# lingo-db/lingo-db

Measured on AMD Instinct MI355X. Metric: tpch_sf100_geomean_ms, lower is better.
Workload: dtype int64/int128 decimal

## Files before the change

lingo-db_amd/csrc/ldb_core.hip:

```cpp
#include "ldb_internal.h"
#include "ldb_device.h"
#include "ldb_chain.h"
#include <algorithm>
#include <cstdlib>
#include <memory>

static thread_local char g_err[1024] = "";
void ldb_set_error(const char* fmt, ...) {
   va_list ap;
   va_start(ap, fmt);
   vsnprintf(g_err, sizeof(g_err), fmt, ap);
   va_end(ap);
}
extern "C" const char* ldb_gpu_last_error(void) { return g_err; }

#include <atomic>
#include <functional>
#include <mutex>
static std::mutex g_opt_mu;
static std::atomic<int64_t> g_option_epoch{0};
static std::unordered_map<std::string, int64_t> g_opts;
int64_t ldb_option(const char* name, int64_t dflt) {
   std::lock_guard<std::mutex> lock(g_opt_mu);
   auto it = g_opts.find(name);
   if (it != g_opts.end()) return it->second;
   std::string env = "LDB_";
   for (const char* c = name; *c; c++) env += (char) toupper((unsigned char) *c);
   int64_t v = dflt;
   if (const char* e = getenv(env.c_str())) v = atoll(e);
   g_opts[name] = v;
   return v;
}
extern "C" int32_t ldb_gpu_set_option(const char* name, int64_t value) {
   if (!name) LDB_FAIL(LDB_ERR_INVALID, "set_option: NULL name");
   static const char* known[] = {"jit", "jit_min_rows", "lazy_filter", "lazy_min_rows", "join_ordered", "join_chained", "gb_ordered", "gb_sorted", "zone_maps", "zone_min_rows", "gb_direct", "gb_wgs_per_cu", "gb_partition", "gb_partition_min_rows", "join_radix", "join_radix_min_rows", "join_radix_min_table_bytes", "join_radix_part_bytes", "probe_batch", "debug_check", "join_direct", "join_rank", "join_coarse", "dict_encode", "dict_min_rows", "comm_transport", "comm_timeout_ms", "desc_cache", "desc_cache_mb", "plan_replay", "scan_single_pass", "lazy_strings", "lazy_strings_min_rows", "gb_partition_wc", "join_radix_wc", "join_radix_lds", "gb_dense_out", "gb_partition_values", "join_pair32", "gb_dense_keys", "jit_async", "jit_threads", "jit_disk_cache", "join_all_match", "topk_short_select", "gb_fits64", "join_coarse_fine", "join_coarse_filtered", "compact_wide_tiles", "compact_max_words", "join_fuse_max_conjuncts", "join_coarse_finest", "jit_min_rows_like", "scan_split", "jit_share_compiles", "scan_strset_min_in"};
   bool ok = false;
   for (const char* k : known) ok |= strcmp(k, name) == 0;
   if (!ok) LDB_FAIL(LDB_ERR_INVALID, "set_option: unknown option '%s'", name);
   std::lock_guard<std::mutex> lock(g_opt_mu);
   g_opts[name] = value;
   g_option_epoch.fetch_add(1);
   return LDB_OK;
}
extern "C" int64_t ldb_gpu_get_option(const char* name) {
   if (!name) return -1;
   std::lock_guard<std::mutex> lock(g_opt_mu);
   auto it = g_opts.find(name);
   if (it != g_opts.end()) return it->second;
   std::string env = "LDB_";
   for (const char* c = name; *c; c++) env += (char) toupper((unsigned char) *c);
   if (const char* e = getenv(env.c_str())) return atoll(e);
   return -1;
}

double ldb_host_trace_threshold() {
   static const double thr = [] {
      const char* e = getenv("LDB_HOST_TRACE");
      return e && *e ? atof(e) : -1.0;
   }();
   return thr;
}
static size_t ldb_size_class(size_t bytes) {
   if (bytes <= 256) return 256;
   const int lg = 63 - __builtin_clzll((unsigned long long) (bytes - 1));
   const size_t step = (size_t) 1 << (lg >= 3 ? lg - 3 : 0);
   return (bytes + step - 1) / step * step;
}
static void ldb_cache_release(ldb_ctx* ctx) {
   for (auto& kv : ctx->parked)
      for (void* p : kv.second) (void) hipFreeAsync(p, ctx->stream);
   ctx->parked.clear();
   ctx->cache_bytes = 0;
}
int32_t ldb_dev_alloc(ldb_ctx* ctx, void** out, size_t bytes) {
   const size_t cls = ctx->cache_on ? ldb_size_class(bytes + 16) : bytes + 16;
   if (ctx->cache_on) {
      auto it = ctx->parked.find(cls);
      if (it != ctx->parked.end() && !it->second.empty()) {
         std::pop_heap(it->second.begin(), it->second.end(), std::greater<void*>());
         *out = it->second.back();
         it->second.pop_back();
         ctx->cache_bytes -= cls;
         ctx->live[*out] = cls;
         return LDB_OK;
      }
   }
   hipError_t e;
   {
      LdbSlow slow_("hipMallocAsync", cls);
      e = hipMallocAsync(out, cls, ctx->stream);
   }
   if (e != hipSuccess && ctx->cache_bytes) {
      (void) hipGetLastError();
      ldb_cache_release(ctx);
      (void) hipStreamSynchronize(ctx->stream);
      e = hipMallocAsync(out, cls, ctx->stream);
   }
   LDB_HIP(e);
   if (ctx->cache_on) ctx->live[*out] = cls;
   return LDB_OK;
}
void ldb_dev_free(ldb_ctx* ctx, void* p) {
   if (!p) return;
   auto dref = ctx->desc_blocks.find(p);
   if (dref != ctx->desc_blocks.end()) {
      if (dref->second > 0) dref->second--;
      else {
         ctx->desc_underflows++;
         if (ldb_host_trace_threshold() >= 0) fprintf(stderr, "[ldb] descriptor %p given back twice\n", p);
      }
      return;
   }
   if (!ctx->shared.empty()) {
      auto sh = ctx->shared.find(p);
      if (sh != ctx->shared.end()) {
         if (--sh->second == 0) ctx->shared.erase(sh);
         return;
      }
// ... 2038 lines not shown
```

lingo-db_amd/csrc/ldb_join.hip:

```cpp
#include "ldb_internal.h"
#include "ldb_join_kernel.h"
#include "ldb_jit.h"
#include <cmath>
#include "ldb_chain.h"
#include <algorithm>
#include <memory>

struct ldb_hashtable {
   ldb_ctx* ctx = nullptr;
   ldb_rel* build = nullptr;
   std::vector<ldb_colref> keys;
   uint64_t* slots = nullptr;
   uint64_t cap = 0;
   int32_t key32 = 0;
   int32_t unique = 0;
   int32_t ordered_slots = 0;
   int64_t kmin = 0, kmax = -1;
   uint64_t kmult = 0;
   uint32_t kmult32 = 0, ksh = 0;
   int32_t slot32 = 0;
   uint32_t* key_bits = nullptr;
   int32_t chained = 0;
   uint32_t* next = nullptr;
   int32_t direct = 0;
// ... 46 lines not shown
   __shared__ uint32_t s_prefix;
   if (threadIdx.x == 0) s_tile = atomicAdd(ticket, 1ull) - ticket_base;
   __syncthreads();
   const uint64_t tile = s_tile;
   const uint64_t base = tile * CHAIN_TILE + (uint64_t) threadIdx.x * CHAIN_ITEMS;
   uint32_t bits[CHAIN_ITEMS];
   uint32_t sum = 0;
#pragma unroll
   for (int k = 0; k < CHAIN_ITEMS; k++) {
      bits[k] = base + k < n_words ? (uint32_t) tab[base + k] : 0u;
      sum += (uint32_t) __popc(bits[k]);
   }
   uint32_t agg;
   uint32_t excl = d_block_scan256<uint32_t>(sum, s_wave, &agg);
   if (threadIdx.x < 64) {
      const uint32_t prefix = d_chain_prefix<uint32_t, 32>(status, tile, epoch, agg, threadIdx.x);
      if (threadIdx.x == 0) s_prefix = prefix;
   }
   __syncthreads();
   excl += s_prefix;
   if (total && tile == n_tiles - 1 && threadIdx.x == 0) *total = (unsigned long long) s_prefix + agg;
#pragma unroll
   for (int k = 0; k < CHAIN_ITEMS; k++) {
      if (base + k < n_words) tab[base + k] = (uint64_t) bits[k] | ((uint64_t) excl << 32);
      excl += (uint32_t) __popc(bits[k]);
   }
}
__global__ void k_join_probe_pairs(const DJoin* __restrict__ d);
__global__ void k_join_probe_pairs_count(const DJoin* __restrict__ d);
__global__ void k_join_probe_count(const DJoin* __restrict__ d);
__global__ void k_join_probe_exists(const DJoin* __restrict__ d);
__global__ void k_join_probe_unique(const DJoin* __restrict__ d);
__global__ void k_join_probe_markbuild(const DJoin* __restrict__ d);
__global__ void k_join_flags_bitmap(const uint8_t* __restrict__ flags, uint64_t n, int anti, uint64_t* __restrict__ bitmap, unsigned long long* __restrict__ counter) {
   join_flags_bitmap_body(flags, n, anti, bitmap, counter);
}
__global__ void k_join_flags_bitmap2(const uint8_t* __restrict__ flags, const uint8_t* __restrict__ not_flags, uint64_t n, uint64_t* __restrict__ bitmap, unsigned long long* __restrict__ counter) {
   join_flags_bitmap_body(flags, n, 0, bitmap, counter, not_flags);
}

static const char* JOIN_SPEC_SRC =
   "extern \"C\" __global__ void k_join_build_spec(const DJoin* __restrict__ d) { join_build_body(LDB_META, d); }\n"
   "extern \"C\" __global__ void k_join_probe_pairs_spec(const DJoin* __restrict__ d) { join_probe_pairs_body(LDB_META, d); }\n"
   "extern \"C\" __global__ void k_join_probe_pairs_count_spec(const DJoin* __restrict__ d) { join_probe_pairs_count_body(LDB_META, d); }\n"
   "extern \"C\" __global__ void k_join_probe_count_spec(const DJoin* __restrict__ d) { join_probe_count_body(LDB_META, d); }\n"
   "extern \"C\" __global__ void k_join_probe_exists_spec(const DJoin* __restrict__ d) { join_probe_exists_body(LDB_META, d); }\n"
   "extern \"C\" __global__ void k_join_probe_unique_spec(const DJoin* __restrict__ d) { join_probe_unique_body(LDB_META, d); }\n"
   "extern \"C\" __global__ void k_join_probe_markbuild_spec(const DJoin* __restrict__ d) { join_probe_markbuild_body(LDB_META, d); }\n";

typedef void (*join_kernel_t)(const DJoin*);
static int32_t launch_join(ldb_ctx* ctx, const DJoin* h, const DJoin* d, int grid, const char* prof_name, const char* spec_name, join_kernel_t generic) {
   hipFunction_t spec = nullptr;
   if (ldb_jit_wanted((int64_t) h->n_rows)) {
      auto meta = std::make_unique<DJoin>();
      memcpy(meta.get(), h, sizeof(DJoin));
      meta->n_rows = meta->cap = meta->slots = meta->out_probe = meta->out_build = meta->out_cap = 0;
      meta->counter = meta->bitmap = meta->mark = meta->mark2 = meta->match = meta->flags = 0;
      meta->kmin = meta->kmax = 0;
      meta->kmult = 0;
      meta->kmult32 = meta->ksh = 0;
      meta->key_bits = 0;
      meta->next = 0;
      meta->coarse = 0;
      meta->coarse_words = 0;
      ldb_jit_strip_keys(meta->bkeys);
      ldb_jit_strip_keys(meta->pkeys);
      for (int p = 0; p < LDB_MAX_PREDS; p++) ldb_jit_strip_pred(meta->ppreds[p]);
      for (int p = 0; p < LDB_MAX_M2PREDS; p++) ldb_jit_strip_pred(meta->m2preds[p]);
      for (int k = 0; k < LDB_MAX_RESID; k++) {
         ldb_jit_strip_col(meta->resid[k].pcol);
         ldb_jit_strip_col(meta->resid[k].bcol);
      }
      std::string why;
      std::string one;
      for (const char* line = JOIN_SPEC_SRC; *line;) {
         const char* nl = strchr(line, '\n');
         const size_t len = nl ? (size_t) (nl - line) + 1 : strlen(line);
         std::string l(line, len);
         if (l.find(std::string(" ") + spec_name + "(") != std::string::npos) one = l;
         line += len;
      }
      spec = ldb_jit_kernel(ctx->device, "ldb_join_kernel.h", "DJoin", one.empty() ? JOIN_SPEC_SRC : one.c_str(), spec_name, meta.get(), sizeof(DJoin), &why);
   }
   const unsigned lds = h->has_coarse ? 4u * h->coarse_words : 0u;
   const bool big_lds = lds > 40u * 1024u;
   const bool tiles = h->n_ppreds > 0;
   const unsigned block = (h->has_coarse && !tiles) ? (big_lds ? 1024u : 512u) : 256u;
   if (h->has_coarse && !tiles) grid = (int) std::max<int64_t>(1, std::min<int64_t>(((int64_t) h->n_rows + block - 1) / block, (int64_t) ctx->cus * (big_lds ? 1 : 4)));
   if (big_lds) {
      if (spec) (void) hipFuncSetAttribute((const void*) spec, hipFuncAttributeMaxDynamicSharedMemorySize, (int) lds);
      else (void) hipFuncSetAttribute((const void*) generic, hipFuncAttributeMaxDynamicSharedMemorySize, (int) lds);
      (void) hipGetLastError();
   }
   LdbProf prof_(ctx, prof_name);
   if (spec) {
      void* params[] = {(void*) &d};
      LDB_HIP(hipModuleLaunchKernel(spec, (unsigned) grid, 1, 1, block, 1, 1, lds, ctx->stream, params, nullptr));
   } else {
      hipLaunchKernelGGL(generic, dim3(grid), dim3(block), lds, ctx->stream, d);
   }
   LDB_HIP(hipGetLastError());
   return LDB_OK;
}

bool ldb_join_jit_check(std::string* log) {
   auto m = std::make_unique<DJoin>();
   memset(m.get(), 0, sizeof(DJoin));
   m->key32 = 1;
   m->kind = LDB_JOIN_INNER;
   m->has_bitmap = 1;
   m->ordered_slots = 1;
   m->has_key_bits = 1;
   m->build_unique = 1;
   m->slot32 = 1;
   m->bkeys.n_keys = m->pkeys.n_keys = 1;
   m->bkeys.cols[0].type = m->pkeys.cols[0].type = LDB_T_INT32;
   m->bkeys.cols[0].width = m->pkeys.cols[0].width = 4;
   m->n_ppreds = 2;
   for (int p = 0; p < 2; p++) {
      m->ppreds[p].col.type = LDB_T_DATE32;
      m->ppreds[p].col.width = 4;
      m->ppreds[p].op = p ? LDB_F_LTE : LDB_F_GTE;
      m->ppreds[p].lo = p ? 9861 : 9131;
      m->ppreds[p].same_col = p;
   }
   if (const char* shape = getenv("LDB_JIT_CHECK_SHAPE")) {
      if (!strcmp(shape, "fk_count")) {
         m->n_ppreds = 0;
         m->has_key_bits = 0;
         m->has_bitmap = 0;
      }
   }
   if (!ldb_jit_compile_only("ldb_join_kernel.h", "DJoin", JOIN_SPEC_SRC, m.get(), sizeof(DJoin), log)) return false;
   m->n_ppreds = 0;
   m->ordered_slots = 0;
   m->slot32 = 0;
   m->has_key_bits = 0;
   m->direct = 1;
   if (!ldb_jit_compile_only("ldb_join_kernel.h", "DJoin", JOIN_SPEC_SRC, m.get(), sizeof(DJoin), log)) return false;
   m->direct = 2;
   m->rank_sorted = 1;
   if (!ldb_jit_compile_only("ldb_join_kernel.h", "DJoin", JOIN_SPEC_SRC, m.get(), sizeof(DJoin), log)) return false;
   m->rank_sorted = 0;
   m->kind = LDB_JOIN_SEMI;
   if (!ldb_jit_compile_only("ldb_join_kernel.h", "DJoin", JOIN_SPEC_SRC, m.get(), sizeof(DJoin), log)) return false;
   m->rank_sorted = 1;
   m->has_coarse = 32 | 6;
   return ldb_jit_compile_only("ldb_join_kernel.h", "DJoin", JOIN_SPEC_SRC, m.get(), sizeof(DJoin), log);
}

__global__ void k_word_pop(const uint64_t* __restrict__ bitmap, uint32_t* __restrict__ pop, uint64_t n_words) {
   for (uint64_t w = blockIdx.x * (uint64_t) blockDim.x + threadIdx.x; w < n_words; w += (uint64_t) gridDim.x * blockDim.x) pop[w] = (uint32_t) __popcll(bitmap[w]);
}
__global__ void k_bitmap_expand(const uint64_t* __restrict__ bitmap, const uint32_t* __restrict__ word_off, uint32_t* __restrict__ out, uint64_t n_words) {
   const uint32_t lane = threadIdx.x & 63;
   const uint64_t wave = (blockIdx.x * (uint64_t) blockDim.x + threadIdx.x) >> 6;
   const uint64_t n_waves = ((uint64_t) gridDim.x * blockDim.x) >> 6;
   for (uint64_t w = wave; w < n_words; w += n_waves) {
      uint64_t m = bitmap[w];
      if ((m >> lane) & 1) out[word_off[w] + d_rank_in(m)] = (uint32_t) (w * 64 + lane);
   }
}
__global__ void k_bitmap_expand_sparse(const uint64_t* __restrict__ bitmap, const uint32_t* __restrict__ word_off, uint32_t* __restrict__ out, uint64_t n_words) {
   for (uint64_t w = blockIdx.x * (uint64_t) blockDim.x + threadIdx.x; w < n_words; w += (uint64_t) gridDim.x * blockDim.x) {
      uint64_t m = bitmap[w];
      if (!m) continue;
      uint32_t at = word_off[w];
      const uint32_t base = (uint32_t) (w * 64);
      while (m) {
         out[at++] = base + (uint32_t) __builtin_ctzll(m);
         m &= m - 1;
      }
   }
}
static void launch_bitmap_expand(ldb_ctx* ctx, const uint64_t* bitmap, const uint32_t* off, uint32_t* out, int64_t n_words, uint64_t total) {
   if (total * 8 < (uint64_t) n_words * 64) hipLaunchKernelGGL(k_bitmap_expand_sparse, dim3(ldb_grid_for(ctx, n_words, 256, 8)), dim3(256), 0, ctx->stream, bitmap, off, out, (uint64_t) n_words);
   else hipLaunchKernelGGL(k_bitmap_expand, dim3(ldb_grid_for(ctx, n_words * 64, 256, 8)), dim3(256), 0, ctx->stream, bitmap, off, out, (uint64_t) n_words);
}
__global__ void k_iota_u32j(uint32_t* out, uint64_t n) {
   for (uint64_t i = blockIdx.x * (uint64_t) blockDim.x + threadIdx.x; i < n; i += (uint64_t) gridDim.x * blockDim.x) out[i] = (uint32_t) i;
}
__global__ void k_unmatched_to_zero(const uint64_t* __restrict__ bitmap, uint32_t* __restrict__ match, uint64_t n) {
   const uint64_t n_words = (n + 63) / 64;
   for (uint64_t w = blockIdx.x * (uint64_t) blockDim.x + threadIdx.x; w < n_words; w += (uint64_t) gridDim.x * blockDim.x) {
      uint64_t missing = ~bitmap[w];
      if (w == n_words - 1 && (n & 63)) missing &= (1ull << (n & 63)) - 1ull;
      while (missing) {
         const int b = __ffsll((unsigned long long) missing) - 1;
         match[w * 64 + (uint64_t) b] = 0u;
         missing &= missing - 1;
      }
   }
}
__global__ void k_compose_null(const uint32_t* __restrict__ ids, const uint32_t* __restrict__ sel, uint32_t* __restrict__ out, uint64_t n) {
   for (uint64_t i = blockIdx.x * (uint64_t) blockDim.x + threadIdx.x; i < n; i += (uint64_t) gridDim.x * blockDim.x) {
      uint32_t s = sel[i];
      out[i] = s == LDB_NULL_ROW ? LDB_NULL_ROW : (ids ? ids[s] : s);
   }
}

__global__ void k_concat_rowids(const uint32_t* __restrict__ first, uint64_t na, const uint32_t* __restrict__ second, uint64_t nb, int pad_nulls, uint32_t* __restrict__ out) {
   for (uint64_t i = blockIdx.x * (uint64_t) blockDim.x + threadIdx.x; i < na + nb; i += (uint64_t) gridDim.x * blockDim.x)
      out[i] = i < na ? (first ? first[i] : (uint32_t) i) : (pad_nulls ? LDB_NULL_ROW : (second ? second[i - na] : (uint32_t) (i - na)));
}

__global__ void k_max_rowid(const uint32_t* __restrict__ ids, uint64_t n, unsigned int* __restrict__ out) {
   unsigned int mx = 0;
   for (uint64_t i = blockIdx.x * (uint64_t) blockDim.x + threadIdx.x; i < n; i += (uint64_t) gridDim.x * blockDim.x) {
      const uint32_t v = ids[i];
      if (v != LDB_NULL_ROW && v > mx) mx = v;
   }
   if (mx) atomicMax(out, mx);
}
static int32_t debug_check_ids(ldb_ctx* ctx, const char* what, const uint32_t* ids, uint64_t n, int64_t limit, const DJoin* h) {
   if (!ids || !n) return LDB_OK;
   unsigned int* d = (unsigned int*) (ctx->d_scratch + 40);
// ... 484 lines not shown
      if (build->n_rows) LDB_TRY(launch_join(ctx, h, d, ldb_grid_for(ctx, build->n_rows, 256, 8), "k_join_build", "k_join_build_spec", k_join_build));
      d_desc.release();
      uint64_t f = 0;
      LDB_TRY(ldb_read_u64_at(ctx, dflags, &f, LDB_SITE, LDB_RB_ORDER_DEPENDENT));
      if (ht->direct && (f & 1) && !ht->chained) {
         ht->chained = 1;
         LDB_TRY(LdbBufs::alloc_into(ctx, &ht->next, 4 * (size_t) build->n_rows));
         LDB_HIP(hipMemsetAsync(ht->slots, 0, ht->slot_bytes, ctx->stream));
         LDB_TRY(ldb_counters(ctx, 1, (uint64_t**) &dflags));
         h->flags = (uint64_t) dflags;
         continue;
      }
      if ((f & 2) && !ht->chained) {
         if (ht->ordered_slots) {
            ht->ordered_slots = 0;
            LdbBufs::drop(ctx, &ht->key_bits);
         } else {
            ht->chained = 1;
            LDB_TRY(LdbBufs::alloc_into(ctx, &ht->next, 4 * (size_t) build->n_rows));
         }
         LDB_HIP(hipMemsetAsync(ht->slots, 0, ht->slot_bytes, ctx->stream));
         LDB_TRY(ldb_counters(ctx, 1, (uint64_t**) &dflags));
         h->flags = (uint64_t) dflags;
         continue;
      }
      if ((f & 1) || ht->chained) ht->unique = 0;
      break;
   }
   *out = ht.release();
   return LDB_OK;
}
extern "C" int32_t ldb_gpu_hashtable_release(ldb_ctx* ctx, ldb_hashtable* ht) {
   (void) ctx;
   delete ht;
   return LDB_OK;
}
extern "C" int64_t ldb_gpu_hashtable_slots(const ldb_hashtable* ht) { return ht ? (int64_t) ht->cap : -1; }
extern "C" int64_t ldb_gpu_hashtable_bytes(const ldb_hashtable* ht) { return ht ? (int64_t) ht->slot_bytes : -1; }

static int32_t make_probe_desc(ldb_hashtable* ht, ldb_rel* probe, const ldb_colref* keys, int32_t n_keys, DJoin* h, const ldb_join_residual* resid = nullptr,
                               int32_t n_resid = 0) {
   if ((size_t) n_keys != ht->keys.size()) LDB_FAIL(LDB_ERR_INVALID, "join_probe: %d probe keys vs %zu build keys", n_keys, ht->keys.size());
   memset(h, 0, sizeof(*h));
   LDB_TRY(ldb_make_dkeys(ht->build, ht->keys.data(), n_keys, &h->bkeys));
   LDB_TRY(ldb_make_dkeys(probe, keys, n_keys, &h->pkeys));
   for (int k = 0; k < n_keys; k++) {
      bool sa = h->bkeys.cols[k].type == LDB_T_UTF8, sb = h->pkeys.cols[k].type == LDB_T_UTF8;
      bool fa = h->bkeys.cols[k].type == LDB_T_FLOAT64 || h->bkeys.cols[k].type == LDB_T_FLOAT32;
      bool fb = h->pkeys.cols[k].type == LDB_T_FLOAT64 || h->pkeys.cols[k].type == LDB_T_FLOAT32;
      if (sa != sb || fa != fb) LDB_FAIL(LDB_ERR_INVALID, "join_probe: key %d type class differs between build and probe", k);
      if ((h->bkeys.cols[k].type == LDB_T_DATE32) != (h->pkeys.cols[k].type == LDB_T_DATE32)) LDB_FAIL(LDB_ERR_INVALID, "join_probe: key %d date vs non-date", k);
      bool wa = h->bkeys.cols[k].type == LDB_T_DECIMAL128 && h->bkeys.cols[k].precision >= 19;
      bool wb = h->pkeys.cols[k].type == LDB_T_DECIMAL128 && h->pkeys.cols[k].precision >= 19;
      if (wa != wb) LDB_FAIL(LDB_ERR_INVALID, "join_probe: key %d decimal width class differs (cast to a common type first)", k);
   }
   h->n_rows = (uint64_t) probe->n_rows;
   h->cap = ht->cap;
   h->slots = (uint64_t) ht->slots;
   h->key32 = ht->key32;
   h->ordered_slots = ht->ordered_slots;
   h->direct = ht->direct;
   h->rank_sorted = ht->rank_sorted;
   h->kmin = ht->kmin;
   h->kmax = ht->kmax;
   h->kmult = ht->kmult;
   h->kmult32 = ht->kmult32;
   h->ksh = ht->ksh;
   h->slot32 = ht->ordered_slots ? ht->slot32 : 0;
   h->key_bits = (uint64_t) ht->key_bits;
   h->has_key_bits = ht->key_bits ? 1 : 0;
   h->chained = ht->chained;
   h->next = (uint64_t) ht->next;
   h->pair32 = 0;
   if (ht->pair32 && !ht->chained) {
      bool narrow = true;
      for (int k = 0; k < 2; k++) {
         const DCol& c = h->pkeys.cols[k];
         narrow = narrow && c.width == 4 && (c.type == LDB_T_INT32 || c.type == LDB_T_DATE32 || c.type == LDB_T_CHAR4);
      }
      h->pair32 = narrow ? 1 : 2;
   }
   h->build_unique = (ht->unique && !ht->chained) ? 1 : 0;
   h->n_ppreds = (int32_t) probe->pending.size();
   if (ht->coarse && probe->n_rows >= (1 << 22) && (probe->pending.empty() || (4u * ht->coarse_words <= 16u * 1024u && ldb_option("join_coarse_filtered", 1) != 0))) {
      h->coarse = (uint64_t) ht->coarse;
      h->coarse_words = ht->coarse_words;
      h->has_coarse = (int32_t) (32u | ht->coarse_shift);
   }
   for (size_t p = 0; p < probe->pending.size(); p++) h->ppreds[p] = probe->pending[p];
   ldb_order_preds(h->ppreds, h->n_ppreds);
   if (n_resid < 0 || n_resid > LDB_MAX_RESID || (n_resid && !resid)) LDB_FAIL(LDB_ERR_UNSUPPORTED, "join_probe: %d residual conjuncts (max %d)", n_resid, LDB_MAX_RESID);
   h->n_resid = n_resid;
   for (int32_t k = 0; k < n_resid; k++) {
      LDB_TRY(ldb_make_dcol(probe, resid[k].probe_col, &h->resid[k].pcol));
      LDB_TRY(ldb_make_dcol(ht->build, resid[k].build_col, &h->resid[k].bcol));
      const int op = resid[k].op;
      if (op < LDB_F_EQ || op > LDB_F_GTE) LDB_FAIL(LDB_ERR_INVALID, "join_probe: residual %d: comparison operator expected", k);
      for (const DCol* c : {&h->resid[k].pcol, &h->resid[k].bcol})
         if (c->type == LDB_T_UTF8 || c->type == LDB_T_FLOAT32 || c->type == LDB_T_FLOAT64) LDB_FAIL(LDB_ERR_UNSUPPORTED, "join_probe: residual %d: integer / decimal / date columns only", k);
      h->resid[k].op = op;
   }
   return LDB_OK;
}

static int32_t probe_count_impl(ldb_ctx* ctx, ldb_hashtable* ht, ldb_rel* probe, const ldb_colref* keys, int32_t n_keys, int64_t* matches, bool radix_ok, const RadixProbe* part = nullptr);
extern "C" int32_t ldb_gpu_join_probe_count(ldb_ctx* ctx, ldb_hashtable* ht, ldb_rel* probe, const ldb_colref* keys, int32_t n_keys, int64_t* matches) {
   return probe_count_impl(ctx, ht, probe, keys, n_keys, matches, true);
}
static int32_t probe_count_impl(ldb_ctx* ctx, ldb_hashtable* ht, ldb_rel* probe, const ldb_colref* keys, int32_t n_keys, int64_t* matches, bool radix_ok, const RadixProbe* part) {
   if (!ctx || !ht || !probe || !matches) LDB_FAIL(LDB_ERR_INVALID, "join_probe_count: NULL argument");
   if (radix_ok) {
      RadixProbe rp(ctx);
      LDB_TRY(radix_prepare(ctx, ht, probe, keys, n_keys, LDB_JOIN_INNER, rp));
      if (rp.rel) {
         const ldb_colref k0 = {0, 0};
         return probe_count_impl(ctx, ht, rp.rel, &k0, 1, matches, false, &rp);
      }
   }
   auto hp = std::make_unique<DJoin>();
   LDB_TRY(make_probe_desc(ht, probe, keys, n_keys, hp.get()));
   hp->kind = LDB_JOIN_INNER;
   unsigned long long* counter;
   LDB_TRY(ldb_counters(ctx, 2, (uint64_t**) &counter));
   hp->counter = (uint64_t) counter;
   LdbDesc<DJoin> d_desc(ctx);
   LDB_TRY(d_desc.upload(hp.get(), sizeof(DJoin)));
   DJoin* d = d_desc.p;
   if (probe->n_rows && part_probe_ok(ht, part, 0)) LDB_TRY(launch_part_probe(ctx, ht, part, probe->n_rows, 0, nullptr, nullptr, counter));
   else if (probe->n_rows) LDB_TRY(launch_join(ctx, hp.get(), d, ldb_grid_for(ctx, probe->n_rows, 256, 8), "k_join_probe_count", "k_join_probe_count_spec", k_join_probe_count));
   uint64_t m = 0;
   LDB_TRY(ldb_read_u64(ctx, counter + 1, &m));
   d_desc.release();
   *matches = (int64_t) m;
   return LDB_OK;
}

extern "C" int32_t ldb_gpu_join_probe(ldb_ctx* ctx, ldb_hashtable* ht, ldb_rel* probe, const ldb_colref* keys, int32_t n_keys, int32_t kind, ldb_rel** out,
                                      ldb_table** mark_out) {
   return ldb_gpu_join_probe_residual(ctx, ht, probe, keys, n_keys, kind, nullptr, 0, out, mark_out);
}

static int32_t probe_impl(ldb_ctx* ctx, ldb_hashtable* ht, ldb_rel* probe, const ldb_colref* keys, int32_t n_keys, int32_t kind, const ldb_join_residual* resid, int32_t n_resid,
                          ldb_rel** out, ldb_table** mark_out, bool radix_ok, const RadixProbe* part = nullptr);
extern "C" int32_t ldb_gpu_join_probe_residual(ldb_ctx* ctx, ldb_hashtable* ht, ldb_rel* probe, const ldb_colref* keys, int32_t n_keys, int32_t kind,
                                               const ldb_join_residual* resid, int32_t n_resid, ldb_rel** out, ldb_table** mark_out) {
   return probe_impl(ctx, ht, probe, keys, n_keys, kind, resid, n_resid, out, mark_out, true);
}
static int32_t select_by_bitmap(ldb_ctx* ctx, ldb_rel* src, const uint64_t* bitmap, int64_t n_words, const void* d_count, uint32_t site, LdbBufs* done, ldb_rel** out) {
   uint64_t total = 0;
   LDB_TRY(ldb_read_u64_at(ctx, d_count, &total, site));
   LdbBufs own(ctx);
   uint32_t* sel;
   LDB_TRY(own.alloc(&sel, 4 * (size_t) (total ? total : 1)));
   if (n_words && total) LDB_TRY(ldb_bitmap_compact(ctx, bitmap, n_words, sel, total, nullptr, nullptr, nullptr));
   if (done) done->free_all();
   own.keep(sel);
   return ldb_rel_select(ctx, src, sel, (int64_t) total, out);
}

static int32_t probe_mark_build(ldb_ctx* ctx, ldb_hashtable* ht, ldb_rel* probe, const ldb_colref* keys, int32_t n_keys, int32_t kind, const ldb_join_residual* resid, int32_t n_resid,
                                const ldb_filter_desc* anti_preds, int32_t n_anti_preds, uint32_t site, ldb_rel** out) {
   auto hb = std::make_unique<DJoin>();
   LDB_TRY(make_probe_desc(ht, probe, keys, n_keys, hb.get(), resid, n_resid));
   hb->kind = kind;
   for (int32_t p = 0; p < n_anti_preds; p++) LDB_TRY(ldb_make_dpred(probe, &anti_preds[p], &hb->m2preds[p]));
   hb->n_m2preds = n_anti_preds;
// ... 312 lines not shown
```

lingo-db_amd/csrc/ldb_join_kernel.h:

```cpp
#pragma once
#include "ldb_keys.h"

#define LDB_MAX_RESID 2
#define LDB_MAX_M2PREDS 2
struct DJoinResid {
   DCol pcol;
   DCol bcol;
   int32_t op;
   int32_t pad;
};
struct DJoin {
   uint64_t n_rows;
   uint64_t cap;
   uint64_t slots;
   uint64_t out_probe;
   uint64_t out_build;
   uint64_t out_cap;
   uint64_t counter;
   uint64_t bitmap;
   uint64_t mark;
   uint64_t mark2;
   uint64_t match;
   uint64_t flags;
   int64_t kmin, kmax;
   uint64_t kmult;
   uint32_t kmult32, ksh;
   uint64_t key_bits;
   uint64_t next;
   uint64_t coarse;
   uint32_t coarse_words, pad_c;
   int32_t key32;
   int32_t kind;
   int32_t has_bitmap, has_mark, has_flags;
   int32_t ordered_slots;
   DKeys bkeys;
   DKeys pkeys;
   int32_t n_ppreds;
   int32_t has_key_bits;
   int32_t chained;
   int32_t build_unique;
   int32_t n_resid;
   int32_t slot32;
   int32_t direct;
   int32_t rank_sorted;
   int32_t has_coarse;
   int32_t pair32;
   DJoinResid resid[LDB_MAX_RESID];
   DPred ppreds[LDB_MAX_PREDS];
   int32_t n_m2preds;
   int32_t pad_m2;
   DPred m2preds[LDB_MAX_M2PREDS];
};

extern __shared__ uint32_t ldb_join_lds[];
__device__ __forceinline__ void d_stage_coarse(const DJoin& m, const DJoin* __restrict__ d) {
   if (!m.has_coarse) return;
   const uint32_t* src = gptr<uint32_t>(d->coarse);
   for (uint32_t i = threadIdx.x; i < d->coarse_words; i += blockDim.x) ldb_join_lds[i] = src[i];
   __syncthreads();
}
__device__ __forceinline__ bool d_coarse_hit(const DJoin& m, uint32_t r) {
   const uint32_t s = (uint32_t) m.has_coarse & 31u;
   return (ldb_join_lds[r >> (s + 5u)] >> ((r >> s) & 31u)) & 1u;
}
__device__ __forceinline__ bool d_probe_pass(const DJoin& m, const DJoin* __restrict__ d, uint64_t i) {
   bool pass = true;
   const int np = m.n_ppreds;
   LDB_UNROLL
   for (int p = 0; p < np; p++)
      if (pass) pass = d_eval_pred(PV(m.ppreds[p], d->ppreds[p]), i);
   return pass;
}

#define JOIN_LONG_RUN 512
__device__ __forceinline__ uint64_t d_join_slot(const DJoin& m, const DJoin* __restrict__ d, uint64_t h, int64_t key, uint64_t mask) {
   if (m.key32 && m.ordered_slots) {
      if (m.slot32) return (uint64_t) __umulhi(((uint32_t) key - (uint32_t) d->kmin) << d->ksh, d->kmult32);
      return (((uint64_t) (key - d->kmin) * d->kmult) >> 32) & mask;
   }
   uint64_t x = h;
   x ^= x >> 33;
   x *= 0xFF51AFD7ED558CCDull;
   x ^= x >> 33;
   return x & mask;
}

__device__ __forceinline__ unsigned long long d_key_pair32(const KV& keys, uint64_t i) {
   const CV a = keys.col(0), b = keys.col(1);
   const uint32_t ka = (uint32_t) d_load_i64(a, d_phys_row(a, i)), kb = (uint32_t) d_load_i64(b, d_phys_row(b, i));
   return (unsigned long long) ka | ((unsigned long long) kb << 32);
}

__device__ __forceinline__ void join_build_body(const DJoin& m, const DJoin* __restrict__ d) {
   const uint64_t n = d->n_rows, mask = d->cap - 1;
   unsigned long long* slots = gptr_mut<unsigned long long>(d->slots);
   const KV bkeys(m.bkeys, d->bkeys);
   if (m.direct) {
      uint32_t* tab = gptr_mut<uint32_t>(d->slots);
      uint32_t* next = gptr_mut<uint32_t>(d->next);
      const CV c = bkeys.col(0);
      for (uint64_t i = blockIdx.x * (uint64_t) blockDim.x + threadIdx.x; i < n; i += (uint64_t) gridDim.x * blockDim.x) {
         const uint32_t row = d_phys_row(c, i);
         if (!d_valid(c, row)) continue;
         const uint64_t r = (uint64_t) (d_load_i64(c, row) - d->kmin);
         if (m.chained) {
            next[i] = atomicExch(&tab[r], (uint32_t) i + 1u);
         } else {
            const uint32_t old = atomicCAS(&tab[r], 0u, (uint32_t) i + 1u);
            if (old != 0 && m.has_flags) {
               uint32_t* f = gptr_mut<uint32_t>(d->flags);
               if ((__hip_atomic_load(f, __ATOMIC_RELAXED, __HIP_MEMORY_SCOPE_AGENT) & 1u) == 0) atomicOr(f, 1u);
            }
         }
      }
      return;
   }
   for (uint64_t i = blockIdx.x * (uint64_t) blockDim.x + threadIdx.x; i < n; i += (uint64_t) gridDim.x * blockDim.x) {
      bool nul;
      uint64_t h = d_hash_keys(bkeys, i, &nul);
      if (nul) continue;
      uint64_t word;
      int64_t key = 0;
      if (m.key32) {
         const CV c = bkeys.col(0);
         key = d_load_i64(c, d_phys_row(c, i));
         word = ((uint64_t) (uint32_t) key << 32) | (uint64_t) ((uint32_t) i + 1u);
      } else {
         word = (h & 0xFFFFFFFF00000000ull) | (uint64_t) ((uint32_t) i + 1u);
      }
      uint64_t pos = d_join_slot(m, d, h, key, mask);
      uint32_t steps = 0;
      if (m.chained) {
         uint32_t* next = gptr_mut<uint32_t>(d->next);
         for (;;) {
// ... 587 lines not shown
   const uint32_t lane = threadIdx.x & 63;
   const uint64_t wave = d_wave_id();
   const uint64_t n_waves = ((uint64_t) gridDim.x * blockDim.x) >> 6;
   const uint32_t* chunk_off = gptr<uint32_t>(d->match);
   uint32_t* out_probe = gptr_mut<uint32_t>(d->out_probe);
   uint32_t* out_build = gptr_mut<uint32_t>(d->out_build);
   const uint64_t out_cap = d->out_cap;
   for (uint64_t w0 = wave * JP_U; w0 < n_chunks; w0 += n_waves * JP_U) {
      uint64_t rows[JP_U], at[JP_U];
      bool act[JP_U];
      uint32_t c[JP_U], emitted[JP_U];
#pragma unroll
      for (int u = 0; u < JP_U; u++) {
         rows[u] = (w0 + u) * 64 + lane;
         act[u] = rows[u] < n;
      }
      d_pairs_of_rows<JP_U>(m, d, rows, act, c);
#pragma unroll
      for (int u = 0; u < JP_U; u++) {
         uint32_t incl = c[u];
         for (int off = 1; off < 64; off <<= 1) {
            uint32_t up = __shfl_up(incl, off);
            if (lane >= (uint32_t) off) incl += up;
         }
         at[u] = (uint64_t) (w0 + u < n_chunks ? chunk_off[w0 + u] : 0u) + (incl - c[u]);
         emitted[u] = 0;
         act[u] = act[u] && c[u] != 0;
      }
      uint32_t again[JP_U];
      d_probe_batch<JP_U>(m, d, rows, act, again, [&](int u, uint32_t brow) {
         if (at[u] + emitted[u] < out_cap) {
            out_probe[at[u] + emitted[u]] = (uint32_t) rows[u];
            out_build[at[u] + emitted[u]] = brow;
         }
         emitted[u]++;
         return m.kind != LDB_JOIN_SINGLE;
      });
#pragma unroll
      for (int u = 0; u < JP_U; u++) {
         if (act[u] && emitted[u] == 0 && at[u] < out_cap) {
            out_probe[at[u]] = (uint32_t) rows[u];
            out_build[at[u]] = LDB_NULL_ROW;
         }
      }
   }
}

__device__ __forceinline__ void join_probe_count_body(const DJoin& m, const DJoin* __restrict__ d) {
   const uint64_t n = d->n_rows;
   d_stage_coarse(m, d);
   unsigned long long local = 0;
   const uint32_t lane = threadIdx.x & 63;
   const uint64_t wave = d_wave_id();
   const uint64_t n_waves = ((uint64_t) gridDim.x * blockDim.x) >> 6;
   const uint64_t n_tiles = (n + 64 * JOIN_BATCH - 1) / (64 * JOIN_BATCH);
   DProbePipe<JOIN_BATCH> pipe;
   pipe.start(m, d, wave * JOIN_BATCH * 64, n_waves * JOIN_BATCH * 64, n);
   auto tile = [&](uint64_t t, auto par) __attribute__((always_inline)) {
      uint64_t rows[JOIN_BATCH];
      bool act[JOIN_BATCH];
      uint32_t mt[JOIN_BATCH];
#pragma unroll
      for (int u = 0; u < JOIN_BATCH; u++) {
         rows[u] = (t * JOIN_BATCH + u) * 64 + lane;
         act[u] = rows[u] < n;
      }
      pipe.step(m, d, t * JOIN_BATCH * 64, n, par);
      d_eval_conj_batch<JOIN_BATCH>(m.ppreds, d->ppreds, m.n_ppreds, rows, act);
      d_probe_batch<JOIN_BATCH>(m, d, rows, act, mt, [](int, uint32_t) { return true; }, pipe.keys(m), pipe.words(m));
#pragma unroll
      for (int u = 0; u < JOIN_BATCH; u++) local += mt[u];
   };
   d_tile_loop<JOIN_BATCH>(m, wave, n_tiles, n_waves, tile);
   for (int off = 32; off > 0; off >>= 1) local += __shfl_down(local, off);
   if (lane == 0 && local) atomicAdd(gptr_mut<unsigned long long>(d->counter) + 1, local);
}

#define JT_BLOCK 256
#define JT_U 8
#define JT_ROWS (JT_BLOCK * JT_U)
#ifndef JT_PB
#define JT_PB 4
#endif
struct JoinTile {
   unsigned short q[JT_ROWS];
   unsigned long long bm[JT_ROWS / 64];
   uint32_t qn;
};
__device__ __forceinline__ void d_tile_filter(const DJoin& m, const DJoin* __restrict__ d, uint64_t base, uint64_t n, JoinTile& st) {
   const uint32_t t = threadIdx.x, lane = t & 63;
   if (t < JT_ROWS / 64) st.bm[t] = 0;
   if (t == 0) st.qn = 0;
   __syncthreads();
   uint64_t rows[JT_U];
   bool pass[JT_U];
#pragma unroll
   for (int u = 0; u < JT_U; u++) {
      rows[u] = base + (uint64_t) u * JT_BLOCK + t;
      pass[u] = rows[u] < n;
   }
   d_eval_conj_batch<JT_U>(m.ppreds, d->ppreds, m.n_ppreds, rows, pass);
#pragma unroll
   for (int u = 0; u < JT_U; u++) {
      const uint64_t mask = __ballot(pass[u]);
      uint32_t b = 0;
      if (mask != 0 && lane == (uint32_t) __builtin_ctzll(mask)) b = atomicAdd(&st.qn, (uint32_t) __popcll(mask));
      b = __shfl(b, mask ? __builtin_ctzll(mask) : 0);
      if (pass[u]) st.q[b + (uint32_t) __popcll(mask & ((1ull << lane) - 1ull))] = (unsigned short) (u * JT_BLOCK + t);
   }
   __syncthreads();
}
template <typename ON_MATCH, typename AFTER>
__device__ __forceinline__ void d_tile_probe(const DJoin& m, const DJoin* __restrict__ d, uint64_t base, JoinTile& st, ON_MATCH on_match, AFTER after) {
#ifdef JT_EXTRA_SYNC
   __syncthreads();
#endif
   const uint32_t qn = st.qn;
   for (uint32_t j0 = 0; j0 < qn; j0 += JT_PB * JT_BLOCK) {
      uint64_t rows[JT_PB];
      uint32_t rel[JT_PB], mt[JT_PB];
      bool act[JT_PB];
#pragma unroll
      for (int u = 0; u < JT_PB; u++) {
         const uint32_t j = j0 + (uint32_t) u * JT_BLOCK + threadIdx.x;
         act[u] = j < qn;
         rel[u] = act[u] ? st.q[j] : 0u;
         rows[u] = base + rel[u];
      }
      d_probe_batch<JT_PB>(m, d, rows, act, mt, [&](int u, uint32_t b) { return on_match(rel[u], b); });
#pragma unroll
      for (int u = 0; u < JT_PB; u++)
         if (act[u]) after(rel[u], mt[u]);
   }
}
template <typename AFTER>
__device__ __forceinline__ void d_tile_probe_first(const DJoin& m, const DJoin* __restrict__ d, uint64_t base, JoinTile& st, AFTER after) {
   const uint32_t qn = st.qn;
   for (uint32_t j0 = 0; j0 < qn; j0 += JT_PB * JT_BLOCK) {
      uint64_t rows[JT_PB];
      uint32_t rel[JT_PB], brow[JT_PB];
      bool act[JT_PB];
#pragma unroll
      for (int u = 0; u < JT_PB; u++) {
         const uint32_t j = j0 + (uint32_t) u * JT_BLOCK + threadIdx.x;
         act[u] = j < qn;
         rel[u] = act[u] ? st.q[j] : 0u;
         rows[u] = base + rel[u];
      }
      d_probe_first<JT_PB>(m, d, rows, act, brow);
#ifdef JOIN_DEBUG_COUNTS
      {
         unsigned long long* dc = gptr_mut<unsigned long long>(d->counter);
         unsigned long long q = 0, hit = 0, inr = 0;
#pragma unroll
         for (int u = 0; u < JT_PB; u++) {
            q += act[u] ? 1 : 0;
            hit += (act[u] && brow[u] != LDB_NULL_ROW) ? 1 : 0;
            if (act[u]) {
               const CV c = KV(m.pkeys, d->pkeys).col(0);
               const int64_t kv = d_load_i64(c, (uint32_t) rows[u]);
               if (kv >= d->kmin && kv <= d->kmax) {
                  const uint64_t r = (uint64_t) (kv - d->kmin);
                  inr += (gptr<uint32_t>(d->key_bits)[r >> 5] >> (r & 31)) & 1u;
               }
            }
         }
         atomicAdd(dc + 2, q);
         atomicAdd(dc + 3, inr);
         atomicAdd(dc + 4, hit);
      }
#endif
#pragma unroll
      for (int u = 0; u < JT_PB; u++)
         if (act[u]) after(rel[u], brow[u]);
   }
}
__device__ __forceinline__ void d_tile_flush(const DJoin* __restrict__ d, uint64_t tile, uint64_t n_words, JoinTile& st, unsigned long long& local) {
   uint64_t* bitmap = gptr_mut<uint64_t>(d->bitmap);
   __syncthreads();
   if (threadIdx.x < JT_ROWS / 64) {
      const uint64_t w = tile * (JT_ROWS / 64) + threadIdx.x;
      if (w < n_words) {
         bitmap[w] = st.bm[threadIdx.x];
         local += (unsigned long long) __popcll(st.bm[threadIdx.x]);
      }
   }
   __syncthreads();
}
__device__ __forceinline__ void d_block_count_add(const DJoin* __restrict__ d, unsigned long long local) {
   if (threadIdx.x < 64) {
      for (int off = 32; off > 0; off >>= 1) local += __shfl_down(local, off);
      if (threadIdx.x == 0 && local) atomicAdd(gptr_mut<unsigned long long>(d->counter), local);
   }
}

__device__ __forceinline__ void join_probe_unique_filtered_body(const DJoin& m, const DJoin* __restrict__ d) {
   __shared__ JoinTile st;
   const uint64_t n = d->n_rows;
   const uint64_t n_words = (n + 63) / 64, n_tiles = (n + JT_ROWS - 1) / JT_ROWS;
   uint32_t* match = gptr_mut<uint32_t>(d->match);
   unsigned long long local = 0;
   for (uint64_t tile = blockIdx.x; tile < n_tiles; tile += gridDim.x) {
      const uint64_t base = tile * JT_ROWS;
      d_tile_filter(m, d, base, n, st);
      d_tile_probe_first(m, d, base, st, [&](uint32_t r, uint32_t b) {
         if (b != LDB_NULL_ROW) {
            match[base + r] = b;
            atomicOr(&st.bm[r >> 6], 1ull << (r & 63));
         }
      });
      d_tile_flush(d, tile, n_words, st, local);
   }
   d_block_count_add(d, local);
}

#define JE_U 4
__device__ __forceinline__ void join_probe_exists_body(const DJoin& m, const DJoin* __restrict__ d) {
   const uint64_t n = d->n_rows;
   d_stage_coarse(m, d);
   if (m.n_ppreds > 0) {
      __shared__ JoinTile st;
      const uint64_t n_words = (n + 63) / 64, n_tiles = (n + JT_ROWS - 1) / JT_ROWS;
      unsigned long long local = 0;
      for (uint64_t tile = blockIdx.x; tile < n_tiles; tile += gridDim.x) {
         const uint64_t base = tile * JT_ROWS;
         d_tile_filter(m, d, base, n, st);
         d_tile_probe_first(m, d, base, st, [&](uint32_t r, uint32_t b) {
            if (m.kind == LDB_JOIN_ANTI ? b == LDB_NULL_ROW : b != LDB_NULL_ROW) atomicOr(&st.bm[r >> 6], 1ull << (r & 63));
         });
         d_tile_flush(d, tile, n_words, st, local);
      }
      d_block_count_add(d, local);
      return;
   }
   const uint64_t n_words = (n + 63) / 64;
   const uint32_t lane = threadIdx.x & 63;
   const uint64_t wave = d_wave_id();
   const uint64_t n_waves = ((uint64_t) gridDim.x * blockDim.x) >> 6;
   uint64_t* bitmap = gptr_mut<uint64_t>(d->bitmap);
   uint8_t* mark = gptr_mut<uint8_t>(d->mark);
   unsigned long long local = 0;
   DProbePipe<JE_U> pipe;
   pipe.start(m, d, wave * JE_U * 64, n_waves * JE_U * 64, n);
   auto tile = [&](uint64_t w0, auto par) __attribute__((always_inline)) {
      uint64_t rows[JE_U];
      bool act[JE_U];
      uint32_t first[JE_U];
#pragma unroll
      for (int u = 0; u < JE_U; u++) {
         rows[u] = (w0 + u) * 64 + lane;
         act[u] = rows[u] < n;
      }
      pipe.step(m, d, w0 * 64, n, par);
      d_probe_first<JE_U>(m, d, rows, act, first, pipe.keys(m), pipe.words(m));
#pragma unroll
      for (int u = 0; u < JE_U; u++) {
         const bool hit = first[u] != LDB_NULL_ROW;
         const bool keep = act[u] && (m.kind == LDB_JOIN_ANTI ? !hit : hit);
         if (m.has_mark && act[u]) mark[rows[u]] = hit ? 1 : 0;
         const uint64_t mm = __ballot(keep);
         if (lane == 0 && w0 + u < n_words) {
            bitmap[w0 + u] = mm;
            local += (unsigned long long) __popcll(mm);
         }
      }
   };
   d_tile_loop<JE_U>(m, wave * JE_U, n_words, n_waves * JE_U, tile);
   if (lane == 0 && local) atomicAdd(gptr_mut<unsigned long long>(d->counter), local);
}

__device__ __forceinline__ void join_probe_markbuild_body(const DJoin& m, const DJoin* __restrict__ d) {
   const uint64_t n = d->n_rows;
   d_stage_coarse(m, d);
   uint8_t* flags = gptr_mut<uint8_t>(d->mark);
   if (m.n_ppreds > 0) {
      __shared__ JoinTile st;
      const uint64_t n_tiles = (n + JT_ROWS - 1) / JT_ROWS;
      for (uint64_t tile = blockIdx.x; tile < n_tiles; tile += gridDim.x) {
         const uint64_t base = tile * JT_ROWS;
         d_tile_filter(m, d, base, n, st);
         d_tile_probe(
            m, d, base, st,
            [&](uint32_t, uint32_t b) {
               flags[b] = 1;
               return true;
            },
            [](uint32_t, uint32_t) {});
         __syncthreads();
      }
      return;
   }
   const uint32_t lane = threadIdx.x & 63;
   const uint64_t wave = d_wave_id();
   const uint64_t n_waves = ((uint64_t) gridDim.x * blockDim.x) >> 6;
   const uint64_t n_tiles = (n + 64 * JE_U - 1) / (64 * JE_U);
   DProbePipe<JE_U> pipe;
   pipe.start(m, d, wave * JE_U * 64, n_waves * JE_U * 64, n);
   auto tile = [&](uint64_t t, auto par) __attribute__((always_inline)) {
      uint64_t rows[JE_U];
      bool act[JE_U];
      uint32_t mt[JE_U];
#pragma unroll
      for (int u = 0; u < JE_U; u++) {
         rows[u] = (t * JE_U + u) * 64 + lane;
         act[u] = rows[u] < n;
      }
      pipe.step(m, d, t * JE_U * 64, n, par);
      d_probe_batch<JE_U>(
         m, d, rows, act, mt,
         [&](int u, uint32_t b) {
            flags[b] = 1;
            if (m.n_m2preds > 0) {
               bool also = true;
               LDB_UNROLL
               for (int p = 0; p < m.n_m2preds; p++)
                  if (also) also = d_eval_pred(PV(m.m2preds[p], d->m2preds[p]), rows[u]);
               if (also) gptr_mut<uint8_t>(d->mark2)[b] = 1;
            }
            return true;
         },
         pipe.keys(m), pipe.words(m));
   };
   d_tile_loop<JE_U>(m, wave, n_tiles, n_waves, tile);
}
__device__ __forceinline__ void join_flags_bitmap_body(const uint8_t* __restrict__ flags, uint64_t n, int anti, uint64_t* __restrict__ bitmap,
                                                       unsigned long long* __restrict__ counter, const uint8_t* __restrict__ not_flags = nullptr) {
   const uint64_t n_words = (n + 63) / 64;
   const uint32_t lane = threadIdx.x & 63;
   const uint64_t wave = d_wave_id();
   const uint64_t n_waves = ((uint64_t) gridDim.x * blockDim.x) >> 6;
   unsigned long long local = 0;
   for (uint64_t w = wave; w < n_words; w += n_waves) {
      const uint64_t i = w * 64 + lane;
      bool keep = i < n && ((flags[i] != 0) != (anti != 0));
      if (not_flags && keep) keep = not_flags[i] == 0;
      uint64_t mm = __ballot(keep);
      if (lane == 0) {
         bitmap[w] = mm;
         local += (unsigned long long) __popcll(mm);
      }
   }
   if (lane == 0 && local) atomicAdd(counter, local);
}

__device__ __forceinline__ void join_probe_unique_body(const DJoin& m, const DJoin* __restrict__ d) {
   d_stage_coarse(m, d);
   if (m.n_ppreds > 0 && m.has_bitmap) {
      join_probe_unique_filtered_body(m, d);
      return;
   }
   const uint64_t n = d->n_rows;
   const uint64_t n_words = (n + 63) / 64;
   const uint32_t lane = threadIdx.x & 63;
   const uint64_t wave = d_wave_id();
   const uint64_t n_waves = ((uint64_t) gridDim.x * blockDim.x) >> 6;
   uint64_t* bitmap = gptr_mut<uint64_t>(d->bitmap);
   uint32_t* match = gptr_mut<uint32_t>(d->match);
   unsigned long long local = 0;
   DProbePipe<JE_U> pipe;
   pipe.start(m, d, wave * JE_U * 64, n_waves * JE_U * 64, n);
   auto tile = [&](uint64_t w0, auto par) __attribute__((always_inline)) {
      uint32_t brow[JE_U];
      uint64_t rows[JE_U];
      bool act[JE_U], pass[JE_U];
#pragma unroll
      for (int u = 0; u < JE_U; u++) {
         rows[u] = (w0 + u) * 64 + lane;
         act[u] = pass[u] = rows[u] < n;
      }
      pipe.step(m, d, w0 * 64, n, par);
      d_eval_conj_batch<JE_U>(m.ppreds, d->ppreds, m.n_ppreds, rows, pass);
// ... 15 lines not shown
```

Measured before the change: 3.588.

## Stage probe join keys into LDS during tile filtering with adaptive toggle

During the filtered tile join path, each tile now loads the 32-bit probe keys with coalesced nontemporal reads while evaluating predicates and writes the keys of surviving rows into LDS next to the row queue. The probe phase then reads keys from LDS instead of doing scattered global gathers. An adaptive mode turns staging off for the next tile when the previous tile's survivor count falls below a threshold, so sparse filters do not pay for reading keys that are never used. The cost is extra LDS, an extra full key-column read when selectivity is low, and more JIT variants.

```diff
diff --git a/lingo-db_amd/csrc/ldb_core.hip b/lingo-db_amd/csrc/ldb_core.hip
--- a/lingo-db_amd/csrc/ldb_core.hip
+++ b/lingo-db_amd/csrc/ldb_core.hip
@@ -33,7 +33,7 @@
 }
 extern "C" int32_t ldb_gpu_set_option(const char* name, int64_t value) {
    if (!name) LDB_FAIL(LDB_ERR_INVALID, "set_option: NULL name");
-   static const char* known[] = {"jit", "jit_min_rows", "lazy_filter", "lazy_min_rows", "join_ordered", "join_chained", "gb_ordered", "gb_sorted", "zone_maps", "zone_min_rows", "gb_direct", "gb_wgs_per_cu", "gb_partition", "gb_partition_min_rows", "join_radix", "join_radix_min_rows", "join_radix_min_table_bytes", "join_radix_part_bytes", "probe_batch", "debug_check", "join_direct", "join_rank", "join_coarse", "dict_encode", "dict_min_rows", "comm_transport", "comm_timeout_ms", "desc_cache", "desc_cache_mb", "plan_replay", "scan_single_pass", "lazy_strings", "lazy_strings_min_rows", "gb_partition_wc", "join_radix_wc", "join_radix_lds", "gb_dense_out", "gb_partition_values", "join_pair32", "gb_dense_keys", "jit_async", "jit_threads", "jit_disk_cache", "join_all_match", "topk_short_select", "gb_fits64", "join_coarse_fine", "join_coarse_filtered", "compact_wide_tiles", "compact_max_words", "join_fuse_max_conjuncts", "join_coarse_finest", "jit_min_rows_like", "scan_split", "jit_share_compiles", "scan_strset_min_in"};
+   static const char* known[] = {"jit", "jit_min_rows", "lazy_filter", "lazy_min_rows", "join_ordered", "join_chained", "gb_ordered", "gb_sorted", "zone_maps", "zone_min_rows", "gb_direct", "gb_wgs_per_cu", "gb_partition", "gb_partition_min_rows", "join_radix", "join_radix_min_rows", "join_radix_min_table_bytes", "join_radix_part_bytes", "probe_batch", "debug_check", "join_direct", "join_rank", "join_coarse", "dict_encode", "dict_min_rows", "comm_transport", "comm_timeout_ms", "desc_cache", "desc_cache_mb", "plan_replay", "scan_single_pass", "lazy_strings", "lazy_strings_min_rows", "gb_partition_wc", "join_radix_wc", "join_radix_lds", "gb_dense_out", "gb_partition_values", "join_pair32", "gb_dense_keys", "jit_async", "jit_threads", "jit_disk_cache", "join_all_match", "topk_short_select", "gb_fits64", "join_coarse_fine", "join_coarse_filtered", "compact_wide_tiles", "compact_max_words", "join_fuse_max_conjuncts", "join_coarse_finest", "jit_min_rows_like", "scan_split", "jit_share_compiles", "scan_strset_min_in", "join_tile_keys", "join_tile_keys_min"};
    bool ok = false;
    for (const char* k : known) ok |= strcmp(k, name) == 0;
    if (!ok) LDB_FAIL(LDB_ERR_INVALID, "set_option: unknown option '%s'", name);
diff --git a/lingo-db_amd/csrc/ldb_join.hip b/lingo-db_amd/csrc/ldb_join.hip
--- a/lingo-db_amd/csrc/ldb_join.hip
+++ b/lingo-db_amd/csrc/ldb_join.hip
@@ -152,9 +152,9 @@
       }
       spec = ldb_jit_kernel(ctx->device, "ldb_join_kernel.h", "DJoin", one.empty() ? JOIN_SPEC_SRC : one.c_str(), spec_name, meta.get(), sizeof(DJoin), &why);
    }
-   const unsigned lds = h->has_coarse ? 4u * h->coarse_words : 0u;
+   const bool tiles = h->n_ppreds > 0;
+   const unsigned lds = (h->has_coarse ? 4u * h->coarse_words : 0u) + (tiles && h->tile_keys ? 4u * (unsigned) JT_QK : 0u);
    const bool big_lds = lds > 40u * 1024u;
-   const bool tiles = h->n_ppreds > 0;
    const unsigned block = (h->has_coarse && !tiles) ? (big_lds ? 1024u : 512u) : 256u;
    if (h->has_coarse && !tiles) grid = (int) std::max<int64_t>(1, std::min<int64_t>(((int64_t) h->n_rows + block - 1) / block, (int64_t) ctx->cus * (big_lds ? 1 : 4)));
    if (big_lds) {
@@ -202,6 +202,14 @@
       }
    }
    if (!ldb_jit_compile_only("ldb_join_kernel.h", "DJoin", JOIN_SPEC_SRC, m.get(), sizeof(DJoin), log)) return false;
+   if (m->n_ppreds > 0) {
+      m->tile_keys = 1;
+      m->tile_keys_min = JT_ROWS / 8;
+      if (!ldb_jit_compile_only("ldb_join_kernel.h", "DJoin", JOIN_SPEC_SRC, m.get(), sizeof(DJoin), log)) return false;
+      m->tile_keys = 2;
+      if (!ldb_jit_compile_only("ldb_join_kernel.h", "DJoin", JOIN_SPEC_SRC, m.get(), sizeof(DJoin), log)) return false;
+      m->tile_keys = m->tile_keys_min = 0;
+   }
    m->n_ppreds = 0;
    m->ordered_slots = 0;
    m->slot32 = 0;
@@ -852,6 +860,14 @@
    }
    h->build_unique = (ht->unique && !ht->chained) ? 1 : 0;
    h->n_ppreds = (int32_t) probe->pending.size();
+   {
+      const DCol& kc = h->pkeys.cols[0];
+      const int64_t mode = ldb_option("join_tile_keys", 1);
+      if (h->n_ppreds > 0 && n_keys == 1 && h->key32 && kc.width == 4 && kc.type != LDB_T_FLOAT32 && !kc.rowids && !kc.validity && (mode == 1 || mode == 2)) {
+         h->tile_keys = (int32_t) mode;
+         h->tile_keys_min = (int32_t) std::max<int64_t>(0, std::min<int64_t>(JT_ROWS + 1, ldb_option("join_tile_keys_min", JT_ROWS / 8)));
+      }
+   }
    if (ht->coarse && probe->n_rows >= (1 << 22) && (probe->pending.empty() || (4u * ht->coarse_words <= 16u * 1024u && ldb_option("join_coarse_filtered", 1) != 0))) {
       h->coarse = (uint64_t) ht->coarse;
       h->coarse_words = ht->coarse_words;
diff --git a/lingo-db_amd/csrc/ldb_join_kernel.h b/lingo-db_amd/csrc/ldb_join_kernel.h
--- a/lingo-db_amd/csrc/ldb_join_kernel.h
+++ b/lingo-db_amd/csrc/ldb_join_kernel.h
@@ -50,6 +50,8 @@
    int32_t n_m2preds;
    int32_t pad_m2;
    DPred m2preds[LDB_MAX_M2PREDS];
+   int32_t tile_keys;
+   int32_t tile_keys_min;
 };
 
 extern __shared__ uint32_t ldb_join_lds[];
@@ -803,22 +805,45 @@
 #ifndef JT_PB
 #define JT_PB 4
 #endif
+#ifndef JT_QK
+#define JT_QK (JT_PB * JT_BLOCK)
+#endif
 struct JoinTile {
    unsigned short q[JT_ROWS];
    unsigned long long bm[JT_ROWS / 64];
    uint32_t qn;
 };
-__device__ __forceinline__ void d_tile_filter(const DJoin& m, const DJoin* __restrict__ d, uint64_t base, uint64_t n, JoinTile& st) {
+static_assert(JT_QK > 0 && JT_QK <= JT_ROWS && JT_QK % (JT_PB * JT_BLOCK) == 0, "JT_QK: whole probe iterations of a tile's queue");
+__device__ __forceinline__ bool d_tile_keys_on(const DJoin& m) {
+   return m.tile_keys != 0 && m.key32 && m.pkeys.cols[0].width == 4 && m.pkeys.cols[0].type != LDB_T_FLOAT32 && !m.pkeys.cols[0].rowids && !m.pkeys.cols[0].validity;
+}
+__device__ __forceinline__ uint32_t* d_tile_qk(const DJoin& m, const DJoin* __restrict__ d) { return ldb_join_lds + (m.has_coarse ? d->coarse_words : 0u); }
+__device__ __forceinline__ bool d_tile_keys_next(const DJoin& m, uint32_t qn) { return d_tile_keys_on(m) && (m.tile_keys == 2 || qn >= (uint32_t) m.tile_keys_min); }
+__device__ __forceinline__ uint32_t d_tile_filter(const DJoin& m, const DJoin* __restrict__ d, uint64_t base, uint64_t n, JoinTile& st, bool stage) {
    const uint32_t t = threadIdx.x, lane = t & 63;
    if (t < JT_ROWS / 64) st.bm[t] = 0;
    if (t == 0) st.qn = 0;
    __syncthreads();
    uint64_t rows[JT_U];
    bool pass[JT_U];
+   uint32_t kv[JT_U];
+   uint32_t* qk = d_tile_qk(m, d);
 #pragma unroll
    for (int u = 0; u < JT_U; u++) {
       rows[u] = base + (uint64_t) u * JT_BLOCK + t;
       pass[u] = rows[u] < n;
+      kv[u] = 0;
+   }
+   if (d_tile_keys_on(m) && stage) {
+      const uint64_t left = n - base;
+      const uint32_t left32 = left > 0xFFFFFFFFull ? 0xFFFFFFFFu : (uint32_t) left;
+      const int32_t* kt = gptr<int32_t>(d->pkeys.cols[0].values) + base;
+#pragma unroll
+      for (int u = 0; u < JT_U; u++) {
+         const uint32_t o = (uint32_t) u * JT_BLOCK + t;
+         kv[u] = (uint32_t) __builtin_nontemporal_load(&kt[o < left32 ? o : 0u]);
+      }
+      asm volatile("" : : : "memory");
    }
    d_eval_conj_batch<JT_U>(m.ppreds, d->ppreds, m.n_ppreds, rows, pass);
 #pragma unroll
@@ -827,19 +852,35 @@
       uint32_t b = 0;
       if (mask != 0 && lane == (uint32_t) __builtin_ctzll(mask)) b = atomicAdd(&st.qn, (uint32_t) __popcll(mask));
       b = __shfl(b, mask ? __builtin_ctzll(mask) : 0);
-      if (pass[u]) st.q[b + (uint32_t) __popcll(mask & ((1ull << lane) - 1ull))] = (unsigned short) (u * JT_BLOCK + t);
+      if (pass[u]) {
+         const uint32_t at = b + (uint32_t) __popcll(mask & ((1ull << lane) - 1ull));
+         st.q[at] = (unsigned short) (u * JT_BLOCK + t);
+         if (d_tile_keys_on(m) && stage && at < JT_QK) qk[at] = kv[u];
+      }
    }
    __syncthreads();
+   return (uint32_t) __builtin_amdgcn_readfirstlane((int) st.qn);
+}
+__device__ __forceinline__ void d_tile_batch_keys(const DJoin& m, const DJoin* __restrict__ d, const JoinTile& st, bool stage, uint32_t j0, const uint64_t (&rows)[JT_PB],
+                                                  const bool (&act)[JT_PB], uint32_t (&kk)[JT_PB]) {
+   const int32_t* kc = gptr<int32_t>(d->pkeys.cols[0].values);
+   const uint32_t* qk = d_tile_qk(m, d);
+   const bool lds = stage && j0 + JT_PB * JT_BLOCK <= JT_QK;
+#pragma unroll
+   for (int u = 0; u < JT_PB; u++) {
+      if (lds) kk[u] = act[u] ? qk[j0 + (uint32_t) u * JT_BLOCK + threadIdx.x] : 0u;
+      else kk[u] = (uint32_t) kc[act[u] ? (uint32_t) rows[u] : 0u];
+   }
 }
 template <typename ON_MATCH, typename AFTER>
-__device__ __forceinline__ void d_tile_probe(const DJoin& m, const DJoin* __restrict__ d, uint64_t base, JoinTile& st, ON_MATCH on_match, AFTER after) {
+__device__ __forceinline__ void d_tile_probe(const DJoin& m, const DJoin* __restrict__ d, uint64_t base, JoinTile& st, bool stage, ON_MATCH on_match, AFTER after) {
 #ifdef JT_EXTRA_SYNC
    __syncthreads();
 #endif
    const uint32_t qn = st.qn;
    for (uint32_t j0 = 0; j0 < qn; j0 += JT_PB * JT_BLOCK) {
       uint64_t rows[JT_PB];
-      uint32_t rel[JT_PB], mt[JT_PB];
+      uint32_t rel[JT_PB], mt[JT_PB], kk[JT_PB];
       bool act[JT_PB];
 #pragma unroll
       for (int u = 0; u < JT_PB; u++) {
@@ -848,18 +889,19 @@
          rel[u] = act[u] ? st.q[j] : 0u;
          rows[u] = base + rel[u];
       }
-      d_probe_batch<JT_PB>(m, d, rows, act, mt, [&](int u, uint32_t b) { return on_match(rel[u], b); });
+      if (d_tile_keys_on(m)) d_tile_batch_keys(m, d, st, stage, j0, rows, act, kk);
+      d_probe_batch<JT_PB>(m, d, rows, act, mt, [&](int u, uint32_t b) { return on_match(rel[u], b); }, d_tile_keys_on(m) ? kk : nullptr);
 #pragma unroll
       for (int u = 0; u < JT_PB; u++)
          if (act[u]) after(rel[u], mt[u]);
    }
 }
 template <typename AFTER>
-__device__ __forceinline__ void d_tile_probe_first(const DJoin& m, const DJoin* __restrict__ d, uint64_t base, JoinTile& st, AFTER after) {
+__device__ __forceinline__ void d_tile_probe_first(const DJoin& m, const DJoin* __restrict__ d, uint64_t base, JoinTile& st, bool stage, AFTER after) {
    const uint32_t qn = st.qn;
    for (uint32_t j0 = 0; j0 < qn; j0 += JT_PB * JT_BLOCK) {
       uint64_t rows[JT_PB];
-      uint32_t rel[JT_PB], brow[JT_PB];
+      uint32_t rel[JT_PB], brow[JT_PB], kk[JT_PB];
       bool act[JT_PB];
 #pragma unroll
       for (int u = 0; u < JT_PB; u++) {
@@ -868,7 +910,8 @@
          rel[u] = act[u] ? st.q[j] : 0u;
          rows[u] = base + rel[u];
       }
-      d_probe_first<JT_PB>(m, d, rows, act, brow);
+      if (d_tile_keys_on(m)) d_tile_batch_keys(m, d, st, stage, j0, rows, act, kk);
+      d_probe_first<JT_PB>(m, d, rows, act, brow, d_tile_keys_on(m) ? kk : nullptr);
 #ifdef JOIN_DEBUG_COUNTS
       {
          unsigned long long* dc = gptr_mut<unsigned long long>(d->counter);
@@ -921,16 +964,18 @@
    const uint64_t n_words = (n + 63) / 64, n_tiles = (n + JT_ROWS - 1) / JT_ROWS;
    uint32_t* match = gptr_mut<uint32_t>(d->match);
    unsigned long long local = 0;
+   bool stage = d_tile_keys_on(m);
    for (uint64_t tile = blockIdx.x; tile < n_tiles; tile += gridDim.x) {
       const uint64_t base = tile * JT_ROWS;
-      d_tile_filter(m, d, base, n, st);
-      d_tile_probe_first(m, d, base, st, [&](uint32_t r, uint32_t b) {
+      const uint32_t qn = d_tile_filter(m, d, base, n, st, stage);
+      d_tile_probe_first(m, d, base, st, stage, [&](uint32_t r, uint32_t b) {
          if (b != LDB_NULL_ROW) {
             match[base + r] = b;
             atomicOr(&st.bm[r >> 6], 1ull << (r & 63));
          }
       });
       d_tile_flush(d, tile, n_words, st, local);
+      stage = d_tile_keys_next(m, qn);
    }
    d_block_count_add(d, local);
 }
@@ -943,13 +988,15 @@
       __shared__ JoinTile st;
       const uint64_t n_words = (n + 63) / 64, n_tiles = (n + JT_ROWS - 1) / JT_ROWS;
       unsigned long long local = 0;
+      bool stage = d_tile_keys_on(m);
       for (uint64_t tile = blockIdx.x; tile < n_tiles; tile += gridDim.x) {
          const uint64_t base = tile * JT_ROWS;
-         d_tile_filter(m, d, base, n, st);
-         d_tile_probe_first(m, d, base, st, [&](uint32_t r, uint32_t b) {
+         const uint32_t qn = d_tile_filter(m, d, base, n, st, stage);
+         d_tile_probe_first(m, d, base, st, stage, [&](uint32_t r, uint32_t b) {
             if (m.kind == LDB_JOIN_ANTI ? b == LDB_NULL_ROW : b != LDB_NULL_ROW) atomicOr(&st.bm[r >> 6], 1ull << (r & 63));
          });
          d_tile_flush(d, tile, n_words, st, local);
+         stage = d_tile_keys_next(m, qn);
       }
       d_block_count_add(d, local);
       return;
@@ -997,17 +1044,19 @@
    if (m.n_ppreds > 0) {
       __shared__ JoinTile st;
       const uint64_t n_tiles = (n + JT_ROWS - 1) / JT_ROWS;
+      bool stage = d_tile_keys_on(m);
       for (uint64_t tile = blockIdx.x; tile < n_tiles; tile += gridDim.x) {
          const uint64_t base = tile * JT_ROWS;
-         d_tile_filter(m, d, base, n, st);
+         const uint32_t qn = d_tile_filter(m, d, base, n, st, stage);
          d_tile_probe(
-            m, d, base, st,
+            m, d, base, st, stage,
             [&](uint32_t, uint32_t b) {
                flags[b] = 1;
                return true;
             },
             [](uint32_t, uint32_t) {});
          __syncthreads();
+         stage = d_tile_keys_next(m, qn);
       }
       return;
    }
```

Measured after the change: 3.614. About the same (+0.7%).
